# jolibrain/joliGEN

Measured on AMD Instinct MI355X. Metric: train images/sec at 256x256 (DDPM UNet step), higher is better.
Workload: dtype bf16; 1 GPU; palette_model DDPM, efficient UNet unet_mha ngf64 mults[1,2,4,8] res_blocks[2,2,2,2] mid-attn 16x32, 256x256, batch 32/GPU, inpainting synthetic masks, AdamW+EMA, iter_size 1 (example_ddpm_noglasses2glasses.json + SURVEY Appendix C overrides); global_batch=32, per_gpu_batch=32, image_size=256, efficient=True, parallelism=dp1, n_ranks_seen=1

## Files before the change

joligen_amd/csrc/common.h:

```cpp
#pragma once
#include <hip/hip_runtime.h>
#include <stdint.h>

#include "../../include/jg355.h"

typedef _Float16 f16_t;
typedef __bf16 bf16_t;
typedef _Float16 f16x8 __attribute__((ext_vector_type(8)));
typedef __bf16 bf16x8 __attribute__((ext_vector_type(8)));
typedef float f32x4 __attribute__((ext_vector_type(4)));
typedef short s16x4_t __attribute__((ext_vector_type(4)));
typedef __attribute__((address_space(3))) s16x4_t* lds_v4;

#define JG_WAVE 64

#define JG_TUNE_LIST(X) \
  X(HALO_CFG, 0) X(WGRAD_HALO_CFG, 0) X(CONV_VARIANT, 6) X(WGRAD_VARIANT, 4) X(SINKHORN_GENERIC, 0) X(CONV1X1, 1) X(GN_REVERSE, 1) \
  X(HALO_DBG, 0) X(PERSIST64, 1) X(HALO_PIPE, 1) X(WGRAD_PIPE, 1) X(CONV_SPLITK, 1) X(CONV_SMALL_TILE, 1) X(GN_FUSED, 1)           \
  X(GN_FUSED_CAP, 256) X(GN_FUSED_DBG, 0) X(GN_FUSED_SLEEP, 4) X(WGRAD_LDS_PAD, 0) X(LN_BWD_CAP, 256) X(DW_BWD_CAP, 512)           \
  X(DW_BWD_PPT, 8) X(CONV_KXK, 1) X(CONV_RING, 1) X(WGRAD_DEEP, 1) X(WGRAD_SW, 0) X(DETERMINISTIC, 0) X(WGRAD_GROUP_BLOCKS, 1024)  \
  X(SGEMM_SPLIT, 0) X(WGRAD_BIG, 1) X(DW_RUN, 1) X(SUBPIXEL_DGRAD_CFG, 0)
#define JG_TUNE_ENUM(name, dflt) JG_TUNE_##name,
enum JgTune { JG_TUNE_LIST(JG_TUNE_ENUM) JG_TUNE_COUNT };
#undef JG_TUNE_ENUM
int jg_tune(int which);
void jg_note_kernel(const char* name);

#define JG_CHECK_LAUNCH()                          \
  do {                                             \
    if (hipGetLastError() != hipSuccess) return JG_ERR_LAUNCH; \
  } while (0)

template <typename T> __device__ __forceinline__ float to_f32(T v) { return (float)v; }
template <typename T> __device__ __forceinline__ T from_f32(float v) { return (T)v; }

template <typename T> __device__ __forceinline__ T bits_to(uint16_t b) { return __builtin_bit_cast(T, b); }
template <typename T> __device__ __forceinline__ uint16_t to_bits(T v) { return __builtin_bit_cast(uint16_t, v); }

template <typename T> __device__ __forceinline__ void unpack8(const uint4& v, float* f) {
  const uint32_t w[4] = {v.x, v.y, v.z, v.w};
#pragma unroll
  for (int i = 0; i < 4; ++i) {
    f[2 * i] = to_f32(bits_to<T>((uint16_t)(w[i] & 0xffffu)));
    f[2 * i + 1] = to_f32(bits_to<T>((uint16_t)(w[i] >> 16)));
  }
}
template <typename T> __device__ __forceinline__ uint4 pack8(const float* f) {
  uint32_t w[4];
#pragma unroll
  for (int i = 0; i < 4; ++i) {
    w[i] = (uint32_t)to_bits<T>(from_f32<T>(f[2 * i])) | ((uint32_t)to_bits<T>(from_f32<T>(f[2 * i + 1])) << 16);
  }
  return make_uint4(w[0], w[1], w[2], w[3]);
}
template <typename T> __device__ __forceinline__ uint2 pack4(float a, float b, float c, float d) {
  uint2 r;
  r.x = (uint32_t)to_bits<T>(from_f32<T>(a)) | ((uint32_t)to_bits<T>(from_f32<T>(b)) << 16);
  r.y = (uint32_t)to_bits<T>(from_f32<T>(c)) | ((uint32_t)to_bits<T>(from_f32<T>(d)) << 16);
  return r;
}
template <typename T> __device__ __forceinline__ void unpack4(const uint2& v, float* f) {
  f[0] = to_f32(bits_to<T>((uint16_t)(v.x & 0xffffu)));
  f[1] = to_f32(bits_to<T>((uint16_t)(v.x >> 16)));
  f[2] = to_f32(bits_to<T>((uint16_t)(v.y & 0xffffu)));
  f[3] = to_f32(bits_to<T>((uint16_t)(v.y >> 16)));
}

template <typename T> struct Mfma;
template <> struct Mfma<f16_t> {
  static __device__ __forceinline__ f32x4 run(const uint4& a, const uint4& b, f32x4 c) {
    return __builtin_amdgcn_mfma_f32_16x16x32_f16(__builtin_bit_cast(f16x8, a), __builtin_bit_cast(f16x8, b), c, 0, 0, 0);
  }
};
template <> struct Mfma<bf16_t> {
  static __device__ __forceinline__ f32x4 run(const uint4& a, const uint4& b, f32x4 c) {
    return __builtin_amdgcn_mfma_f32_16x16x32_bf16(__builtin_bit_cast(bf16x8, a), __builtin_bit_cast(bf16x8, b), c, 0, 0, 0);
  }
};

template <typename T> __device__ __forceinline__ uint4 ldg16(const T* ptr, bool ok) {
  uint4 v = *reinterpret_cast<const uint4*>(ptr);
  v.x = ok ? v.x : 0u;
  v.y = ok ? v.y : 0u;
  v.z = ok ? v.z : 0u;
  v.w = ok ? v.w : 0u;
  return v;
}

__device__ __forceinline__ float sigmoid_fast(float u) { return __builtin_amdgcn_rcpf(1.0f + __expf(-u)); }
__device__ __forceinline__ float silu_f(float u) { return u * sigmoid_fast(u); }
__device__ __forceinline__ float silu_grad_f(float u) {
  const float s = sigmoid_fast(u);
  return s * (1.0f + u * (1.0f - s));
}

template <int ACT> __device__ __forceinline__ float act_f(float u) {
  if (ACT == JG_ACT_SILU) return silu_f(u);
  if (ACT == JG_ACT_RELU) return fmaxf(u, 0.f);
  if (ACT == JG_ACT_LRELU) return u > 0.f ? u : 0.2f * u;
  return u;
}
template <int ACT> __device__ __forceinline__ float act_grad_f(float u) {
  if (ACT == JG_ACT_SILU) return silu_grad_f(u);
  if (ACT == JG_ACT_RELU) return u > 0.f ? 1.f : 0.f;
  if (ACT == JG_ACT_LRELU) return u > 0.f ? 1.f : 0.2f;
  return 1.f;
}
__device__ __forceinline__ float act_grad_rt(float u, int act) {
  return act == JG_ACT_SILU ? silu_grad_f(u) : act == JG_ACT_RELU ? (u > 0.f ? 1.f : 0.f) : act == JG_ACT_LRELU ? (u > 0.f ? 1.f : 0.2f) : 1.f;
}

#define JG_DISPATCH_ACT(act, ...)                          \
  do {                                                     \
    if ((act) == JG_ACT_SILU) { constexpr int ACT = JG_ACT_SILU; __VA_ARGS__ }        \
    else if ((act) == JG_ACT_RELU) { constexpr int ACT = JG_ACT_RELU; __VA_ARGS__ }   \
    else if ((act) == JG_ACT_LRELU) { constexpr int ACT = JG_ACT_LRELU; __VA_ARGS__ } \
    else { constexpr int ACT = JG_ACT_NONE; __VA_ARGS__ }                              \
  } while (0)

__device__ __forceinline__ float wave_sum(float v) {
#pragma unroll
  for (int o = 32; o > 0; o >>= 1) v += __shfl_xor(v, o);
  return v;
}
__device__ __forceinline__ float wave_max(float v) {
#pragma unroll
  for (int o = 32; o > 0; o >>= 1) v = fmaxf(v, __shfl_xor(v, o));
  return v;
}

#define JG_DISPATCH_DTYPE(dtype, ...)                 \
  do {                                                \
    if ((dtype) == JG_F16) {                          \
      typedef f16_t T;                                \
      __VA_ARGS__                                     \
    } else if ((dtype) == JG_BF16) {                  \
      typedef bf16_t T;                               \
      __VA_ARGS__                                     \
    } else {                                          \
      return JG_ERR_BAD_ARG;                          \
    }                                                 \
  } while (0)
```

joligen_amd/csrc/conv1x1.hip:

```cpp
#include <stdlib.h>

#include "conv_params.h"

namespace {

__device__ __forceinline__ float act_rt(float u, int act) {
  return act == JG_ACT_SILU ? silu_f(u) : act == JG_ACT_RELU ? fmaxf(u, 0.f) : act == JG_ACT_LRELU ? (u > 0.f ? u : 0.2f * u) : u;
}

template <typename T, int PAIRS, int KS, bool APPLY = false, bool GNB = false>
__global__ __launch_bounds__(256, 2) void conv1x1_stream_kernel(ConvP p, int ntiles) {
  __shared__ __attribute__((aligned(16))) float s_ab[APPLY ? 4 * 2 * KS * 32 : (GNB ? 4 * 5 * PAIRS * 32 : 4)];
  const int lane = threadIdx.x & 63;
  const int a = lane & 15, g = lane >> 4;
  const int n0 = blockIdx.y * (PAIRS * 32);
  const T* __restrict__ x = (const T*)p.x;
  const T* __restrict__ w = (const T*)p.w;
  const T* __restrict__ res = (const T*)p.res;
  T* __restrict__ y = (T*)p.y;

  uint4 wf[PAIRS][2][KS];
#pragma unroll
  for (int pr = 0; pr < PAIRS; ++pr)
#pragma unroll
    for (int hf = 0; hf < 2; ++hf) {
      const int n = n0 + pr * 32 + (a >> 2) * 8 + hf * 4 + (a & 3);
#pragma unroll
      for (int ks = 0; ks < KS; ++ks) wf[pr][hf][ks] = *reinterpret_cast<const uint4*>(w + (long)n * p.ldw + ks * 32 + g * 8);
    }
  float bs[PAIRS][8];
#pragma unroll
  for (int pr = 0; pr < PAIRS; ++pr)
#pragma unroll
    for (int j = 0; j < 8; ++j) bs[pr][j] = (!GNB && p.bias) ? p.bias[n0 + pr * 32 + g * 8 + j] : 0.f;

  const int wave = blockIdx.x * 4 + (threadIdx.x >> 6), nwaves = gridDim.x * 4;
  auto load_tile = [&](int t, uint4* xf) {
    const T* px = x + ((long)t * 16 + a) * p.ldx + g * 8;
#pragma unroll
    for (int ks = 0; ks < KS; ++ks) xf[ks] = *reinterpret_cast<const uint4*>(px + ks * 32);
  };
  const bool do_apply = APPLY && blockIdx.y == 0;
  float* wab = s_ab + (threadIdx.x >> 6) * (APPLY ? 2 * KS * 32 : (GNB ? 5 * PAIRS * 32 : 1));
  const int tiles_per_img = (p.Ho * p.Wo) >> 4;
  int cur_b = -1;
  constexpr int PF = KS <= 2 ? 4 : (KS <= 4 ? 2 : 1);
  uint4 ring[PF][KS];
#pragma unroll
  for (int s = 0; s < PF; ++s)
    if (wave + s * nwaves < ntiles) load_tile(wave + s * nwaves, ring[s]);
  for (int base = wave; base < ntiles; base += PF * nwaves) {
#pragma unroll
    for (int s = 0; s < PF; ++s) {
      const int t = base + s * nwaves;
      if (t >= ntiles) break;
      const long prow = ((long)t * 16 + a);
      if (GNB) {
        const int b = t / tiles_per_img;
        if (b != cur_b) {
          cur_b = b;
          constexpr int NC = PAIRS * 32;
          for (int c = lane; c < NC; c += 64) {
            const long row = (long)b * p.N + n0 + c;
            wab[c] = p.bab[row * 2];
            wab[NC + c] = p.bab[row * 2 + 1];
            wab[2 * NC + c] = p.bpqr[row * 3];
            wab[3 * NC + c] = p.bpqr[row * 3 + 1];
            wab[4 * NC + c] = p.bpqr[row * 3 + 2];
          }
        }
      }
      uint4 rf[PAIRS];
      if (res) {
#pragma unroll
        for (int pr = 0; pr < PAIRS; ++pr) rf[pr] = *reinterpret_cast<const uint4*>(res + prow * p.ldres + n0 + pr * 32 + g * 8);
      }
      f32x4 acc[PAIRS][2];
#pragma unroll
      for (int pr = 0; pr < PAIRS; ++pr) {
        acc[pr][0] = acc[pr][1] = (f32x4){0.f, 0.f, 0.f, 0.f};
#pragma unroll
        for (int ks = 0; ks < KS; ++ks) {
          acc[pr][0] = Mfma<T>::run(wf[pr][0][ks], ring[s][ks], acc[pr][0]);
          acc[pr][1] = Mfma<T>::run(wf[pr][1][ks], ring[s][ks], acc[pr][1]);
        }
      }
      if (do_apply) {
        const int b = t / tiles_per_img;
        if (b != cur_b) {
          cur_b = b;
          const float* src = p.aab + (long)b * (2 * KS * 32);
          for (int i = lane; i < 2 * KS * 32 / 4; i += 64) reinterpret_cast<float4*>(wab)[i] = reinterpret_cast<const float4*>(src)[i];
        }
        T* ay = (T*)p.ay + prow * p.lday + g * 8;
#pragma unroll
        for (int ks = 0; ks < KS; ++ks) {
          float f[8];
          unpack8<T>(ring[s][ks], f);
          const float4* c4 = reinterpret_cast<const float4*>(wab + (ks * 32 + g * 8) * 2);
#pragma unroll
          for (int k4 = 0; k4 < 4; ++k4) {
            const float4 c = c4[k4];
            const float u0 = c.x * f[2 * k4] + c.y, u1 = c.z * f[2 * k4 + 1] + c.w;
            f[2 * k4] = p.aact == JG_ACT_SILU ? silu_f(u0) : act_rt(u0, p.aact);
            f[2 * k4 + 1] = p.aact == JG_ACT_SILU ? silu_f(u1) : act_rt(u1, p.aact);
          }
          *reinterpret_cast<uint4*>(ay + ks * 32) = pack8<T>(f);
        }
      }
      const int tn = t + PF * nwaves;
      if (tn < ntiles) load_tile(tn, ring[s]);
#pragma unroll
      for (int pr = 0; pr < PAIRS; ++pr) {
        float o[8] = {acc[pr][0][0], acc[pr][0][1], acc[pr][0][2], acc[pr][0][3], acc[pr][1][0], acc[pr][1][1], acc[pr][1][2], acc[pr][1][3]};
        float r8[8];
        if (res) unpack8<T>(rf[pr], r8);
#pragma unroll
        for (int j = 0; j < 8; ++j) o[j] = GNB ? p.alpha * o[j] : p.alpha * o[j] + bs[pr][j] + (res ? p.res_scale * r8[j] : 0.f);
        if (GNB) {
          constexpr int NC = PAIRS * 32;
          const int cl = pr * 32 + g * 8, cg = n0 + cl;
          float fx[8], fd[8], ca[8], cb[8], cP[8], cQ[8], cR[8];
          unpack8<T>(*reinterpret_cast<const uint4*>((const T*)p.bgx + prow * p.bldgx + cg), fx);
          unpack8<T>(*reinterpret_cast<const uint4*>((const T*)p.bgdy + prow * p.bldgdy + cg), fd);
#pragma unroll
          for (int h = 0; h < 2; ++h) {
            *reinterpret_cast<float4*>(ca + 4 * h) = *reinterpret_cast<const float4*>(wab + cl + 4 * h);
            *reinterpret_cast<float4*>(cb + 4 * h) = *reinterpret_cast<const float4*>(wab + NC + cl + 4 * h);
            *reinterpret_cast<float4*>(cP + 4 * h) = *reinterpret_cast<const float4*>(wab + 2 * NC + cl + 4 * h);
            *reinterpret_cast<float4*>(cQ + 4 * h) = *reinterpret_cast<const float4*>(wab + 3 * NC + cl + 4 * h);
            *reinterpret_cast<float4*>(cR + 4 * h) = *reinterpret_cast<const float4*>(wab + 4 * NC + cl + 4 * h);
          }
#pragma unroll
          for (int j = 0; j < 8; ++j) {
            float du = fd[j];
            if (p.bact != JG_ACT_NONE) du *= act_grad_rt(ca[j] * fx[j] + cb[j], p.bact);
            o[j] += du * cP[j] + fx[j] * cQ[j] + cR[j];
          }
          if (p.badd1) {
            float fa[8];
            unpack8<T>(*reinterpret_cast<const uint4*>((const T*)p.badd1 + prow * p.bldadd1 + cg), fa);
#pragma unroll
            for (int j = 0; j < 8; ++j) o[j] += p.bsc1 * fa[j];
          }
          if (p.badd2) {
            float fa[8];
            unpack8<T>(*reinterpret_cast<const uint4*>((const T*)p.badd2 + prow * p.bldadd2 + cg), fa);
#pragma unroll
            for (int j = 0; j < 8; ++j) o[j] += p.bsc2 * fa[j];
          }
        }
        *reinterpret_cast<uint4*>(y + prow * p.ldy + n0 + pr * 32 + g * 8) = pack8<T>(o);
        if (GNB) __builtin_amdgcn_sched_barrier(0);
      }
    }
  }
}

template <typename T, int PAIRS>
__global__ __launch_bounds__(256, 2) void conv3x3_c8_stream_kernel(ConvP p, int ntiles) {
  constexpr int KS = 3;
  const int lane = threadIdx.x & 63;
  const int a = lane & 15, g = lane >> 4;
  const int n0 = blockIdx.y * (PAIRS * 32);
  const T* __restrict__ x = (const T*)p.x;
  const T* __restrict__ w = (const T*)p.w;
  const T* __restrict__ res = (const T*)p.res;
  T* __restrict__ y = (T*)p.y;
  const uint4 zero4 = make_uint4(0u, 0u, 0u, 0u);
  uint4 wf[PAIRS][2][KS];
#pragma unroll
  for (int pr = 0; pr < PAIRS; ++pr)
#pragma unroll
    for (int hf = 0; hf < 2; ++hf) {
      const int n = n0 + pr * 32 + (a >> 2) * 8 + hf * 4 + (a & 3);
#pragma unroll
      for (int ks = 0; ks < KS; ++ks) {
        const int tap = ks * 4 + g;
        wf[pr][hf][ks] = tap < 9 ? *reinterpret_cast<const uint4*>(w + (long)n * p.ldw + tap * 8) : zero4;
      }
    }
  float bs[PAIRS][8];
#pragma unroll
  for (int pr = 0; pr < PAIRS; ++pr)
#pragma unroll
    for (int j = 0; j < 8; ++j) bs[pr][j] = p.bias ? p.bias[n0 + pr * 32 + g * 8 + j] : 0.f;
  const int wave = blockIdx.x * 4 + (threadIdx.x >> 6), nwaves = gridDim.x * 4;
  auto load_tile = [&](int t, uint4* xf) {
    const long pix = (long)t * 16 + a;
    const int px = pix % p.W, py = (pix / p.W) % p.H;
#pragma unroll
    for (int ks = 0; ks < KS; ++ks) {
      const int tap = ks * 4 + g;
      const int dy = tap / 3 - 1, dx = tap % 3 - 1;
      const bool ok = tap < 9 && (unsigned)(py + dy) < (unsigned)p.H && (unsigned)(px + dx) < (unsigned)p.W;
      xf[ks] = ok ? *reinterpret_cast<const uint4*>(x + (pix + (long)dy * p.W + dx) * 8) : zero4;
    }
  };
  const int per = (ntiles + nwaves - 1) / nwaves;
  const int t0 = wave * per, t1 = min(ntiles, t0 + per);
  const int tiles_per_img = (p.H * p.W) >> 4;
  float s1[PAIRS][8], s2[PAIRS][8];
#pragma unroll
  for (int pr = 0; pr < PAIRS; ++pr)
#pragma unroll
    for (int j = 0; j < 8; ++j) s1[pr][j] = s2[pr][j] = 0.f;
  int cur_b = t0 < t1 ? t0 / tiles_per_img : 0;
  auto flush = [&](int b) {
    float* base = p.stats + ((long)(b * p.nslots + wave % p.nslots) * p.ldstats) * 2;
#pragma unroll
    for (int pr = 0; pr < PAIRS; ++pr)
#pragma unroll
      for (int j = 0; j < 8; ++j) {
        float u = s1[pr][j], v = s2[pr][j];
#pragma unroll
        for (int o = 1; o < 16; o <<= 1) {
          u += __shfl_xor(u, o);
          v += __shfl_xor(v, o);
        }
        if (a == 0) {
          atomicAdd(base + (n0 + pr * 32 + g * 8 + j) * 2, u);
          atomicAdd(base + (n0 + pr * 32 + g * 8 + j) * 2 + 1, v);
        }
        s1[pr][j] = s2[pr][j] = 0.f;
      }
  };
  constexpr int PF = 2;
  uint4 ring[PF][KS];
#pragma unroll
  for (int s = 0; s < PF; ++s)
    if (t0 + s < t1) load_tile(t0 + s, ring[s]);
  for (int base = t0; base < t1; base += PF) {
#pragma unroll
    for (int s = 0; s < PF; ++s) {
      const int t = base + s;
      if (t < t1) {
        const long prow = ((long)t * 16 + a);
        if (p.stats) {
          const int b = t / tiles_per_img;
          if (b != cur_b) {
            flush(cur_b);
            cur_b = b;
          }
        }
        f32x4 acc[PAIRS][2];
#pragma unroll
        for (int pr = 0; pr < PAIRS; ++pr) {
          acc[pr][0] = acc[pr][1] = (f32x4){0.f, 0.f, 0.f, 0.f};
#pragma unroll
          for (int ks = 0; ks < KS; ++ks) {
            acc[pr][0] = Mfma<T>::run(wf[pr][0][ks], ring[s][ks], acc[pr][0]);
            acc[pr][1] = Mfma<T>::run(wf[pr][1][ks], ring[s][ks], acc[pr][1]);
          }
        }
        if (t + PF < t1) load_tile(t + PF, ring[s]);
#pragma unroll
        for (int pr = 0; pr < PAIRS; ++pr) {
          float o[8] = {acc[pr][0][0], acc[pr][0][1], acc[pr][0][2], acc[pr][0][3], acc[pr][1][0], acc[pr][1][1], acc[pr][1][2], acc[pr][1][3]};
          float r8[8];
          if (res) unpack8<T>(*reinterpret_cast<const uint4*>(res + prow * p.ldres + n0 + pr * 32 + g * 8), r8);
#pragma unroll
          for (int j = 0; j < 8; ++j) {
            o[j] = p.alpha * o[j] + bs[pr][j] + (res ? p.res_scale * r8[j] : 0.f);
            s1[pr][j] += o[j];
            s2[pr][j] += o[j] * o[j];
          }
          *reinterpret_cast<uint4*>(y + prow * p.ldy + n0 + pr * 32 + g * 8) = pack8<T>(o);
        }
      }
    }
  }
  if (p.stats && t0 < t1) flush(cur_b);
}

template <typename T>
void launch_c8(const ConvP& p, hipStream_t st) {
  const int ntiles = p.M / 16;
  const int ngroups = p.N / 64;
  int bx = (ntiles + 3) / 4;
  const int cap = 256 * 8 / ngroups > 64 ? 256 * 8 / ngroups : 64;
  if (bx > cap) bx = cap;
  jg_note_kernel("conv3x3_c8_stream_kernel");
  hipLaunchKernelGGL((conv3x3_c8_stream_kernel<T, 2>), dim3(bx, ngroups), dim3(256), 0, st, p, ntiles);
}


template <typename T, int PAIRS, int KS>
void launch_1x1(const ConvP& p, hipStream_t st) {
  const int ntiles = p.M / 16;
  const int ngroups = p.N / (PAIRS * 32);
  int bx = (ntiles + 3) / 4;
  const int cap = 256 * 8 / ngroups > 64 ? 256 * 8 / ngroups : 64;
  if (bx > cap) bx = cap;
  if (p.aab) {
    jg_note_kernel("conv1x1_stream_kernel+gn_apply");
    hipLaunchKernelGGL((conv1x1_stream_kernel<T, PAIRS, KS, true>), dim3(bx, ngroups), dim3(256), 0, st, p, ntiles);
  } else if (p.bgx) {
    jg_note_kernel("conv1x1_stream_kernel+gn_bwd_apply");
    hipLaunchKernelGGL((conv1x1_stream_kernel<T, PAIRS, KS, false, true>), dim3(bx, ngroups), dim3(256), 0, st, p, ntiles);
  } else {
    jg_note_kernel("conv1x1_stream_kernel");
    hipLaunchKernelGGL((conv1x1_stream_kernel<T, PAIRS, KS>), dim3(bx, ngroups), dim3(256), 0, st, p, ntiles);
  }
}

template <typename T, int PAIRS, int KS>
void launch_1x1_plain(const ConvP& p, hipStream_t st) {
  const int ntiles = p.M / 16;
  const int ngroups = p.N / (PAIRS * 32);
  int bx = (ntiles + 3) / 4;
  const int cap = 256 * 8 / ngroups > 64 ? 256 * 8 / ngroups : 64;
  if (bx > cap) bx = cap;
  jg_note_kernel("conv1x1_stream_kernel");
  hipLaunchKernelGGL((conv1x1_stream_kernel<T, PAIRS, KS>), dim3(bx, ngroups), dim3(256), 0, st, p, ntiles);
}

template <typename T>
bool dispatch_1x1(const ConvP& p, hipStream_t st) {
  const int ks = p.Cin / 32;
  const bool wide = p.N % 128 == 0;
  if (!p.aab && !p.bgx) {
    if (ks == 1) {
      if (wide) launch_1x1_plain<T, 4, 1>(p, st);
      else if (p.N % 64 == 0) launch_1x1_plain<T, 2, 1>(p, st);
      else launch_1x1_plain<T, 1, 1>(p, st);
      return true;
    }
    if (p.N % 64) {
      switch (ks) {
        case 2: launch_1x1_plain<T, 1, 2>(p, st); return true;
        case 4: launch_1x1_plain<T, 1, 4>(p, st); return true;
        case 8: launch_1x1_plain<T, 1, 8>(p, st); return true;
        default: return false;
      }
    }
  } else if (ks == 1 || p.N % 64) {
    return false;
  }
  switch (ks) {
    case 2: wide ? launch_1x1<T, 4, 2>(p, st) : launch_1x1<T, 2, 2>(p, st); return true;
    case 4: launch_1x1<T, 2, 4>(p, st); return true;
    case 6: launch_1x1<T, 2, 6>(p, st); return true;
    case 8: launch_1x1<T, 2, 8>(p, st); return true;
    default: return false;
  }
}

}

bool jg_conv1x1_try(int dtype, const ConvP& p, int nbatch, hipStream_t st) {
  if (p.res_up || p.x_up || p.y_pool) return false;
  const bool off = jg_tune(JG_TUNE_CONV1X1) == 0;
  if (off && !p.aab && !p.bgx) return false;
  if (!p.aab && !p.bgx && nbatch == 1 && p.nh == 1 && p.R == 3 && p.S == 3 && p.pad == 1 && p.stride == 1 && !p.out_f32 && !(p.stats && p.stats_mode) && !p.reflect &&
      p.Cin == 8 && ((p.H * p.W) & 15) == 0 &&
      p.ldx == 8 && p.ldw == 72 && p.N % 64 == 0 && !(p.M & 15) && p.H == p.Ho && p.W == p.Wo && p.ldy % 8 == 0 && (!p.res || p.ldres % 8 == 0) &&
      (long)p.M >= 65536) {
    if (dtype == JG_F16) launch_c8<f16_t>(p, st);
    else if (dtype == JG_BF16) launch_c8<bf16_t>(p, st);
    else return false;
    return true;
  }
  if (nbatch != 1 || p.nh != 1 || p.R != 1 || p.S != 1 || p.pad != 0 || p.stride != 1 || p.out_f32 || p.stats || p.reflect) return false;
  if (p.Cin % 32 || p.Cin > 256 || p.N % 32 || (p.M & 15)) return false;
  if (p.ldx % 8 || p.ldy % 8 || p.ldw % 8 || (p.res && p.ldres % 8)) return false;
  if ((long)p.M < 65536) return false;
  if (!p.aab && !p.bgx && p.Cin >= 256 && p.N >= 256 && jg_tune(JG_TUNE_CONV1X1) < 2) return false;
  if (dtype == JG_F16) return dispatch_1x1<f16_t>(p, st);
  if (dtype == JG_BF16) return dispatch_1x1<bf16_t>(p, st);
  return false;
}
```

Measured before the change: 680.8 images/sec.

## Add LDS-resident weight slab 1x1 conv kernel with wide column slabs

```diff
diff --git a/joligen_amd/csrc/common.h b/joligen_amd/csrc/common.h
--- a/joligen_amd/csrc/common.h
+++ b/joligen_amd/csrc/common.h
@@ -19,7 +19,7 @@
   X(HALO_DBG, 0) X(PERSIST64, 1) X(HALO_PIPE, 1) X(WGRAD_PIPE, 1) X(CONV_SPLITK, 1) X(CONV_SMALL_TILE, 1) X(GN_FUSED, 1)           \
   X(GN_FUSED_CAP, 256) X(GN_FUSED_DBG, 0) X(GN_FUSED_SLEEP, 4) X(WGRAD_LDS_PAD, 0) X(LN_BWD_CAP, 256) X(DW_BWD_CAP, 512)           \
   X(DW_BWD_PPT, 8) X(CONV_KXK, 1) X(CONV_RING, 1) X(WGRAD_DEEP, 1) X(WGRAD_SW, 0) X(DETERMINISTIC, 0) X(WGRAD_GROUP_BLOCKS, 1024)  \
-  X(SGEMM_SPLIT, 0) X(WGRAD_BIG, 1) X(DW_RUN, 1) X(SUBPIXEL_DGRAD_CFG, 0)
+  X(SGEMM_SPLIT, 0) X(WGRAD_BIG, 1) X(DW_RUN, 1) X(SUBPIXEL_DGRAD_CFG, 0) X(CONV1X1_COLS, 1)
 #define JG_TUNE_ENUM(name, dflt) JG_TUNE_##name,
 enum JgTune { JG_TUNE_LIST(JG_TUNE_ENUM) JG_TUNE_COUNT };
 #undef JG_TUNE_ENUM
diff --git a/joligen_amd/csrc/conv1x1.hip b/joligen_amd/csrc/conv1x1.hip
--- a/joligen_amd/csrc/conv1x1.hip
+++ b/joligen_amd/csrc/conv1x1.hip
@@ -157,6 +157,168 @@
   }
 }
 
+template <typename T, int KS, int WAVES, bool APPLY, bool GNB>
+__global__ __launch_bounds__(WAVES * 64) void conv1x1_cols_kernel(ConvP p, int ntiles, int ns) {
+  extern __shared__ uint4 s_cols[];
+  const int lane = threadIdx.x & 63, wv = threadIdx.x >> 6;
+  const int a = lane & 15, g = lane >> 4;
+  const int n0 = blockIdx.y * ns;
+  const int nsl = min(ns, p.N - n0), np = nsl >> 5;
+  const T* __restrict__ x = (const T*)p.x;
+  const T* __restrict__ w = (const T*)p.w;
+  const T* __restrict__ res = (const T*)p.res;
+  T* __restrict__ y = (T*)p.y;
+  uint4* s_w = s_cols;
+  float* s_c = reinterpret_cast<float*>(s_cols + (ns >> 5) * 2 * KS * 64);
+  float* s_ab = s_c + ns;
+
+  for (int i = threadIdx.x; i < np * 2 * KS * 64; i += WAVES * 64) {
+    const int fr = i >> 6, l = i & 63;
+    const int ks = fr % KS, hf = (fr / KS) & 1, pr = fr / (2 * KS);
+    const int n = n0 + pr * 32 + ((l & 15) >> 2) * 8 + hf * 4 + (l & 3);
+    s_w[i] = *reinterpret_cast<const uint4*>(w + (long)n * p.ldw + ks * 32 + (l >> 4) * 8);
+  }
+  if (!GNB)
+    for (int c = threadIdx.x; c < nsl; c += WAVES * 64) s_c[c] = p.bias ? p.bias[n0 + c] : 0.f;
+  __syncthreads();
+
+  const int stride = gridDim.x * WAVES;
+  auto load_tile = [&](int t, uint4* xf) {
+    const T* px = x + ((long)t * 16 + a) * p.ldx + g * 8;
+#pragma unroll
+    for (int ks = 0; ks < KS; ++ks) xf[ks] = *reinterpret_cast<const uint4*>(px + ks * 32);
+  };
+  const bool do_apply = APPLY && blockIdx.y == 0;
+  const int tiles_per_img = (p.Ho * p.Wo) >> 4;
+  int cur_b = -1;
+  constexpr int PF = KS <= 2 ? 4 : (KS <= 4 ? 2 : 1);
+  uint4 ring[PF][KS];
+#pragma unroll
+  for (int s = 0; s < PF; ++s)
+    if (blockIdx.x * WAVES + s * stride < ntiles) load_tile(blockIdx.x * WAVES + s * stride + wv, ring[s]);
+  const uint4* wl = s_w + lane;
+  for (int base = blockIdx.x * WAVES; base < ntiles; base += PF * stride) {
+#pragma unroll
+    for (int s = 0; s < PF; ++s) {
+      const int tg = base + s * stride;
+      if (tg >= ntiles) break;
+      const int t = tg + wv;
+      const long prow = ((long)t * 16 + a);
+      if (GNB || do_apply) {
+        const int b = tg / tiles_per_img;
+        if (b != cur_b) {
+          cur_b = b;
+          __syncthreads();
+          if (GNB) {
+            for (int c = threadIdx.x; c < nsl; c += WAVES * 64) {
+              const long row = (long)b * p.N + n0 + c;
+              s_c[c] = p.bab[row * 2];
+              s_c[nsl + c] = p.bab[row * 2 + 1];
+              s_c[2 * nsl + c] = p.bpqr[row * 3];
+              s_c[3 * nsl + c] = p.bpqr[row * 3 + 1];
+              s_c[4 * nsl + c] = p.bpqr[row * 3 + 2];
+            }
+          } else {
+            const float* src = p.aab + (long)b * (2 * KS * 32);
+            for (int i = threadIdx.x; i < 2 * KS * 32 / 4; i += WAVES * 64) reinterpret_cast<float4*>(s_ab)[i] = reinterpret_cast<const float4*>(src)[i];
+          }
+          __syncthreads();
+        }
+      }
+      if (do_apply) {
+        T* ay = (T*)p.ay + prow * p.lday + g * 8;
+#pragma unroll
+        for (int ks = 0; ks < KS; ++ks) {
+          float f[8];
+          unpack8<T>(ring[s][ks], f);
+          const float4* c4 = reinterpret_cast<const float4*>(s_ab + (ks * 32 + g * 8) * 2);
+#pragma unroll
+          for (int k4 = 0; k4 < 4; ++k4) {
+            const float4 c = c4[k4];
+            const float u0 = c.x * f[2 * k4] + c.y, u1 = c.z * f[2 * k4 + 1] + c.w;
+            f[2 * k4] = p.aact == JG_ACT_SILU ? silu_f(u0) : act_rt(u0, p.aact);
+            f[2 * k4 + 1] = p.aact == JG_ACT_SILU ? silu_f(u1) : act_rt(u1, p.aact);
+          }
+          *reinterpret_cast<uint4*>(ay + ks * 32) = pack8<T>(f);
+        }
+      }
+      uint4 nx[4];
+      auto request = [&](int pr, uint4* o) {
+        const int cg = n0 + pr * 32 + g * 8;
+        if (GNB) {
+          o[0] = *reinterpret_cast<const uint4*>((const T*)p.bgx + prow * p.bldgx + cg);
+          o[1] = *reinterpret_cast<const uint4*>((const T*)p.bgdy + prow * p.bldgdy + cg);
+          if (p.badd1) o[2] = *reinterpret_cast<const uint4*>((const T*)p.badd1 + prow * p.bldadd1 + cg);
+          if (p.badd2) o[3] = *reinterpret_cast<const uint4*>((const T*)p.badd2 + prow * p.bldadd2 + cg);
+        } else if (res) {
+          o[0] = *reinterpret_cast<const uint4*>(res + prow * p.ldres + cg);
+        }
+      };
+      request(0, nx);
+      for (int pr = 0; pr < np; ++pr) {
+        uint4 cu[4];
+#pragma unroll
+        for (int i = 0; i < (GNB ? 4 : 1); ++i) cu[i] = nx[i];
+        if (pr + 1 < np) request(pr + 1, nx);
+        f32x4 acc0 = (f32x4){0.f, 0.f, 0.f, 0.f}, acc1 = acc0;
+        const uint4* wp = wl + pr * (2 * KS * 64);
+#pragma unroll
+        for (int ks = 0; ks < KS; ++ks) {
+          acc0 = Mfma<T>::run(wp[ks * 64], ring[s][ks], acc0);
+          acc1 = Mfma<T>::run(wp[(KS + ks) * 64], ring[s][ks], acc1);
+        }
+        if (pr == np - 1) {
+          const int tn = t + PF * stride;
+          if (tn < ntiles) load_tile(tn, ring[s]);
+        }
+        const int cl = pr * 32 + g * 8;
+        float o[8] = {acc0[0], acc0[1], acc0[2], acc0[3], acc1[0], acc1[1], acc1[2], acc1[3]};
+        if (GNB) {
+          float fx[8], fd[8], ca[8], cb[8], cP[8], cQ[8], cR[8];
+#pragma unroll
+          for (int j = 0; j < 8; ++j) o[j] = p.alpha * o[j];
+          unpack8<T>(cu[0], fx);
+          unpack8<T>(cu[1], fd);
+#pragma unroll
+          for (int h = 0; h < 2; ++h) {
+            *reinterpret_cast<float4*>(ca + 4 * h) = *reinterpret_cast<const float4*>(s_c + cl + 4 * h);
+            *reinterpret_cast<float4*>(cb + 4 * h) = *reinterpret_cast<const float4*>(s_c + nsl + cl + 4 * h);
+            *reinterpret_cast<float4*>(cP + 4 * h) = *reinterpret_cast<const float4*>(s_c + 2 * nsl + cl + 4 * h);
+            *reinterpret_cast<float4*>(cQ + 4 * h) = *reinterpret_cast<const float4*>(s_c + 3 * nsl + cl + 4 * h);
+            *reinterpret_cast<float4*>(cR + 4 * h) = *reinterpret_cast<const float4*>(s_c + 4 * nsl + cl + 4 * h);
+          }
+#pragma unroll
+          for (int j = 0; j < 8; ++j) {
+            float du = fd[j];
+            if (p.bact != JG_ACT_NONE) du *= act_grad_rt(ca[j] * fx[j] + cb[j], p.bact);
+            o[j] += du * cP[j] + fx[j] * cQ[j] + cR[j];
+          }
+          if (p.badd1) {
+            float fa[8];
+            unpack8<T>(cu[2], fa);
+#pragma unroll
+            for (int j = 0; j < 8; ++j) o[j] += p.bsc1 * fa[j];
+          }
+          if (p.badd2) {
+            float fa[8];
+            unpack8<T>(cu[3], fa);
+#pragma unroll
+            for (int j = 0; j < 8; ++j) o[j] += p.bsc2 * fa[j];
+          }
+        } else {
+          float r8[8], bs[8];
+          if (res) unpack8<T>(cu[0], r8);
+          *reinterpret_cast<float4*>(bs) = *reinterpret_cast<const float4*>(s_c + cl);
+          *reinterpret_cast<float4*>(bs + 4) = *reinterpret_cast<const float4*>(s_c + cl + 4);
+#pragma unroll
+          for (int j = 0; j < 8; ++j) o[j] = p.alpha * o[j] + bs[j] + (res ? p.res_scale * r8[j] : 0.f);
+        }
+        *reinterpret_cast<uint4*>(y + prow * p.ldy + n0 + cl) = pack8<T>(o);
+      }
+    }
+  }
+}
+
 template <typename T, int PAIRS>
 __global__ __launch_bounds__(256, 2) void conv3x3_c8_stream_kernel(ConvP p, int ntiles) {
   constexpr int KS = 3;
@@ -315,10 +477,64 @@
   hipLaunchKernelGGL((conv1x1_stream_kernel<T, PAIRS, KS>), dim3(bx, ngroups), dim3(256), 0, st, p, ntiles);
 }
 
+constexpr int COLS_WAVES = 8;
+constexpr int COLS_LDS = 160 * 1024;
+
+template <typename T, int KS, bool APPLY, bool GNB>
+bool launch_cols_ks(const ConvP& p, hipStream_t st) {
+  auto kern = conv1x1_cols_kernel<T, KS, COLS_WAVES, APPLY, GNB>;
+  const int K = KS * 32;
+  const int per_pair = 32 * (K * 2 + (GNB ? 20 : 4));
+  const int fixed = APPLY ? 2 * K * 4 : 0;
+  const int pairs = p.N / 32, max_pairs = (COLS_LDS - fixed) / per_pair;
+  const int nslabs = (pairs + max_pairs - 1) / max_pairs;
+  const int ns = (pairs + nslabs - 1) / nslabs * 32;
+  const int lds = ns / 32 * per_pair + fixed;
+  static bool attr_set = false;
+  if (!attr_set) {
+    if (hipFuncSetAttribute(reinterpret_cast<const void*>(kern), hipFuncAttributeMaxDynamicSharedMemorySize, COLS_LDS) != hipSuccess) {
+      (void)hipGetLastError();
+      return false;
+    }
+    attr_set = true;
+  }
+  const int ntiles = p.M / 16;
+  const int per_cu = 2 * lds <= COLS_LDS ? 2 : 1;
+  int bx = 256 * per_cu / nslabs;
+  if (bx > ntiles / COLS_WAVES) bx = ntiles / COLS_WAVES;
+  jg_note_kernel(APPLY ? "conv1x1_stream_kernel+gn_apply" : GNB ? "conv1x1_stream_kernel+gn_bwd_apply" : "conv1x1_stream_kernel");
+  hipLaunchKernelGGL(kern, dim3(bx, nslabs), dim3(COLS_WAVES * 64), lds, st, p, ntiles, ns);
+  return true;
+}
+
+template <typename T>
+bool launch_cols(const ConvP& p, hipStream_t st) {
+  const int ks = p.Cin / 32;
+  const bool fused = p.aab || p.bgx;
+  if (fused ? (ks == 1 || p.N % 64) : (p.N % 64 && ks == 6)) return false;
+  const int gw = p.N % 64 ? 32 : (p.N % 128 == 0 && (ks == 2 || (ks == 1 && !fused)) ? 128 : 64);
+  if (p.N / gw < 2) return false;
+  if (p.M % (16 * COLS_WAVES) || (fused && (p.Ho * p.Wo) % (16 * COLS_WAVES))) return false;
+#define JG_COLS_KS(KS_)                                                        \
+  case KS_:                                                                    \
+    return p.aab ? launch_cols_ks<T, KS_, true, false>(p, st)                  \
+                 : p.bgx ? launch_cols_ks<T, KS_, false, true>(p, st) : launch_cols_ks<T, KS_, false, false>(p, st);
+  switch (ks) {
+    case 1: return launch_cols_ks<T, 1, false, false>(p, st);
+    JG_COLS_KS(2)
+    JG_COLS_KS(4)
+    JG_COLS_KS(6)
+    JG_COLS_KS(8)
+    default: return false;
+  }
+#undef JG_COLS_KS
+}
+
 template <typename T>
 bool dispatch_1x1(const ConvP& p, hipStream_t st) {
   const int ks = p.Cin / 32;
   const bool wide = p.N % 128 == 0;
+  if (jg_tune(JG_TUNE_CONV1X1_COLS) == 1 && launch_cols<T>(p, st)) return true;
   if (!p.aab && !p.bgx) {
     if (ks == 1) {
       if (wide) launch_1x1_plain<T, 4, 1>(p, st);
```

New measurement: 687.5 images/sec, median of 6. Within noise of the previous version (+1.0%).
